# bmorris3/gadfly

Hardware: AMD Instinct MI355X
Metric: GP log-likelihood evals/sec (N=1e6, J=30) (higher is better)
Workload: dtype f64

## Files before the change

gadfly_amd/csrc/gadfly_hip.hip:

```cpp

#include <hip/hip_runtime.h>
#include <atomic>
#include <utility>
#include <type_traits>
#include <stdint.h>
#include <stdio.h>
#include <stdarg.h>
#include <math.h>

#include "../../include/gadfly_hip.h"
#include "gf_internal.h"

#define FM_INLINE __device__ __forceinline__
#include "fastmath.h"
#include "gf_wave.h"
#include "gf_sweep.h"

template <unsigned long long BITS>
__device__ __forceinline__ double fm_local_constant(const int z) {
    return __hiloint2double((int)(unsigned)(BITS >> 32) ^ z, (int)(unsigned)(BITS & 0xffffffffull) ^ z);
}
#define GF_K(x) fm_local_constant<__builtin_bit_cast(unsigned long long, (double)(x))>(fm_z)
__device__ __forceinline__ double fm_exp_local(const double x) {
    int fm_z;
// ... 822 lines not shown
constexpr int RED_NACC = 3;
constexpr int RED_BLOCK = 256;
constexpr int RED_MAXG = 512;

__host__ __device__ inline int red_groups(int64_t N) {
    int64_t g = (N + 4095) / 4096;
    if (g < 1) g = 1;
    if (g > RED_MAXG) g = RED_MAXG;
    return (int)g;
}

__device__ inline int64_t steady_rows_stored(const double *steady, int b, int64_t N, int64_t n_first) {
    const double swd = steady[(size_t)b * ST_SIZE + ST_SW];
    if (!(swd > 0.0)) return N;
    const int64_t r = (int64_t)swd - n_first;
    return r < 0 ? 0 : (r < N ? r : N);
}

__device__ __forceinline__ void red_row(const double dn, double &s1, double &mn) {
    s1 += log(dn);
    mn = fmin(mn, dn);
}
__device__ __forceinline__ void red_row_z(const double dn, const double zn, double &s2) { s2 += zn * zn / dn; }

__device__ __forceinline__ void steady_tile_sums(const double *dp, const double *zp, const int64_t N, const int64_t lim,
                                                 double *acc, const int init, const int lane) {
    if (lim == 0 && !init) return;
    const int G = red_groups(N);
    const int64_t gl = (lim + RED_BLOCK - 1) / RED_BLOCK;
    const int Gn = gl < G ? (int)gl : G;
    double a1 = 0.0, a2 = 0.0, am = INFINITY;
#pragma unroll 1
    for (int g = 0; g < Gn; ++g) {
        double t1 = 0.0, t2 = 0.0, t3 = INFINITY;
#pragma unroll 1
        for (int w = 0; w < RED_BLOCK / 64; ++w) {
            double s1 = 0.0, s2 = 0.0, mn = INFINITY;
#pragma unroll 1
            for (int64_t n = (int64_t)g * RED_BLOCK + 64 * w + lane; n < lim; n += (int64_t)G * RED_BLOCK) {
                const double dn = dp[n];
                red_row(dn, s1, mn);
                red_row_z(dn, zp[n], s2);
            }
            wave_sum2(s1, s2);
            mn = -wave_max(-mn);
            t1 += s1;
            t2 += s2;
            t3 = fmin(t3, mn);
        }
        if (lane == (g & 63)) {
            a1 += t1;
            a2 += t2;
            am = fmin(am, t3);
        }
    }
    wave_sum2(a1, a2);
    am = -wave_max(-am);
    if (lane == 0) {
        if (!init) { a1 += acc[0]; a2 += acc[1]; am = fmin(am, acc[2]); }
        acc[0] = a1; acc[1] = a2; acc[2] = am;
    }
}

template <int ROWS, bool ROWSTORE, bool SAMPLE = false, bool STEADY = false>
__global__ void __launch_bounds__(64, 2)
k_factor7(const int64_t N, const int64_t n_first, const int64_t chunk_len, const int nch,
          const int ch0, const int nsel, const int Jr, const int Jc, const int block_sub, const double gap,
          const double *__restrict__ ar_, const double *__restrict__ cr_,
          const double *__restrict__ ac_, const double *__restrict__ bc_,
          const double *__restrict__ cc_, const double *__restrict__ dc_,
          const double *__restrict__ diag_add_, const double *__restrict__ cmax_,
          const double *__restrict__ t_, const int64_t t_bs,
          const double *__restrict__ diag_, const int64_t diag_bs,
          const double *__restrict__ y_, const int64_t y_bs,
          double *__restrict__ d_, double *__restrict__ z_, double *__restrict__ r_out,
          double *__restrict__ Ut_out, double *__restrict__ Wt_out, double *__restrict__ de_out,
          double *__restrict__ S_state, double *__restrict__ F_state,
          int32_t *__restrict__ info, double *__restrict__ steady_, const int64_t arm_from,
          double *acc_, const int acc_init) {
    static_assert(!STEADY || (!ROWSTORE && !SAMPLE), "steady mode: the streamed log-likelihood only");
    const int lane = threadIdx.x;
    const int g = lane >> 5, c = lane & 31;
    const int sel = blockIdx.x;
    const int pr = sel / nsel, ch = ch0 + (sel - pr * nsel);
    const int b = pr * nch + ch;
    int64_t tile_lim = 0;
#define STEADY_EXIT(lim) do { if constexpr (STEADY) { if (acc_) { tile_lim = (lim); goto tile_sums; } } return; } while (0)
  {
    if (info[b] != 0) STEADY_EXIT(steady_rows_stored(steady_, pr, N, n_first));
    double *__restrict__ hdr = STEADY ? steady_ + (size_t)pr * ST_SIZE : nullptr;
    if constexpr (STEADY) { if (hdr[ST_SW] > 0.0) STEADY_EXIT(steady_rows_stored(steady_, pr, N, n_first)); }
    const int64_t c0 = (int64_t)ch * chunk_len;
    const int64_t rows = (N - c0 < chunk_len) ? (N - c0) : chunk_len;
    const int64_t g0 = n_first + c0;
    const size_t pb = (size_t)pr * N + c0;
    const double *__restrict__ tg = t_ + (size_t)pr * t_bs + g0;
    const double *__restrict__ yg = y_ + (size_t)pr * y_bs + g0;
    const bool has_g = diag_ != nullptr;
    const double *__restrict__ gg = has_g ? diag_ + (size_t)pr * diag_bs + g0 : yg;
    double *__restrict__ dg = d_ + pb;
    double *__restrict__ zg = SAMPLE ? z_ + (size_t)pr * y_bs + g0 : z_ + pb;
    const int own = 2 * c + g;
    double *__restrict__ rg = (ROWSTORE && r_out) ? r_out + pb * 64 + own : nullptr;
    double *__restrict__ ug = (ROWSTORE && Ut_out) ? Ut_out + pb * 64 + own : nullptr;
    double *__restrict__ wg = (ROWSTORE && Wt_out) ? Wt_out + pb * 64 + own : nullptr;
    const bool st_ok = own < ROWS || Wt_out != nullptr;
    double *__restrict__ eg = (ROWSTORE && de_out) ? de_out + pb : nullptr;
    double *__restrict__ Sg = S_state + (size_t)b * (64 * 64);
    double *__restrict__ Fg = F_state + (size_t)b * 64;
    const double diag_add = diag_add_[pr];

    RowGen G;
    G.init(own, pr, Jr, Jc, block_sub, gap, ar_, cr_, ac_, bc_, cc_, dc_, cmax_, tg, g0);
    const double cj = G.cj;

    __shared__ __attribute__((aligned(16))) double s_w[64];
    __shared__ __attribute__((aligned(16))) double s_u[64];
    __shared__ __attribute__((aligned(16))) double s_e[64];
    const double2 *pw = (const double2 *)s_w + g, *pu = (const double2 *)s_u + g;
    const double2 *pe = (const double2 *)s_e + g;
    const bool f31 = c == 31;
    const bool fl = lane == 63;
    const double not63 = fl ? 0.0 : 1.0, is31 = f31 ? 1.0 : 0.0;

    double *__restrict__ col0 = Sg + (size_t)(2 * c) * 64 + 2 * g;
    double *__restrict__ col1 = (f31 ? Fg : Sg + (size_t)(2 * c + 1) * 64) + 2 * g;
    double T[ROWS / 2][2];
    const bool zero_start = (block_sub >> 30) & 1;
    constexpr double thr = ST_THR;
    int cnt = 0, fill = 0;
    if constexpr (STEADY) {
        cnt = __builtin_amdgcn_readfirstlane((int)hdr[ST_CNT]);
        fill = __builtin_amdgcn_readfirstlane((int)hdr[ST_FILL]);
    }
#pragma unroll
    for (int m = 0; m < ROWS / 2; ++m) {
        T[m][0] = zero_start ? 0.0 : col0[4 * (m >> 1) + (m & 1)];
        T[m][1] = zero_start ? 0.0 : col1[4 * (m >> 1) + (m & 1)];
    }
    double q0 = 0.0, q1 = 0.0;
    int32_t fail = 0;

    double t_n1 = tg[1], t_n2 = tg[2];
    double y_n = yg[0], y_n1 = yg[1];
    double g_n = gg[0], g_n1 = gg[1];
    double ut, vt, de;
    bool rst;
    G.next(tg[0], g0, ut, vt, rst, de);

    double2 ub[S7_AHEAD + 1], wb[S7_AHEAD + 1];
    s_w[own] = 0.0;
    s_u[own] = ut;
    wave_lds_fence();
    sweep7_preload<ROWS>(ub, wb, pu, pw);

    int64_t n = 0;
    for (; n < rows; ++n) {
        const double a_n = (has_g ? g_n : 0.0) + diag_add, yy = y_n;
        const double ut_c = ut, vt_c = vt;
        const bool rst_c = rst;
        if constexpr (ROWSTORE) { if (eg && lane == 0) eg[n] = rst ? de : -1.0; }
        if (rst) {
            const double el = fm_exp(-cj * de);
            s_e[own] = el;
            wave_lds_fence();
            double d0, d1, el0, el1;
            both_halves(el, el0, el1);
            sweep7_preload<ROWS>(ub, wb, pe, pw);
            sweep7_run<ROWS, true>(T, ub, wb, pe, pw, q0, q1, el0, el1, d0, d1);
            sweep7_preload<ROWS>(ub, wb, pu, pw);
            q0 = 0.0;
            q1 = 0.0;
        }
        __builtin_amdgcn_s_setprio(0);
        double acc0, acc1;
        sweep7_run<ROWS, false>(T, ub, wb, pu, pw, q0, q1, 0.0, 0.0, acc0, acc1);
        __builtin_amdgcn_s_setprio(GF_CHAIN_PRIO);
        const double tmp = own_column_sum(acc0, acc1);
        const double r = (vt_c - tmp) * not63;
        double r0, r1;
        both_halves(r, r0, r1);
        G.next(t_n1, g0 + n + 1, ut, vt, rst, de);
        t_n1 = t_n2; y_n = y_n1; g_n = g_n1;
        t_n2 = tg[n + 3];
        y_n1 = yg[n + 2];
        g_n1 = gg[n + 2];
        wave_lds_fence();
        s_w[own] = r;
        s_u[own] = ut;
        wave_lds_fence();
        sweep7_preload<ROWS>(ub, wb, pu, pw);
        const double s1 = wave_sum(ut_c * tmp);
        const double s2 = read_lane(tmp, 63);
        const double dn = a_n - s1;
        const double zn = SAMPLE ? __dsqrt_rn(dn) * yy : yy - s2;
        if (!(dn > 0.0)) {
            const int64_t gf = g0 + n + 1;
            fail = (int32_t)(gf > 0x7fffffff ? 0x7fffffff : gf);
            break;
        }
        const double inv = fast_rcp(dn);
        q0 = r0 * inv;
        q1 = fma(zn, is31, r1) * inv;
        if constexpr (ROWSTORE) {
            const size_t ro = opaque_uniform((size_t)n * 64);
            if (st_ok) {
                if (rg) rg[ro] = r;
                if (ug) ug[ro] = ut_c;
                if (wg) wg[ro] = r * inv;
            }
        }
        if (lane == 0) { dg[n] = dn; zg[n] = SAMPLE ? zn + s2 : zn; }
        if constexpr (STEADY) {
            const int64_t gn = g0 + n;
            if (rst_c && gn >= arm_from && (gn & (ST_GRID - 1)) == 0) {
                double cs, sn;
                both_halves(vt_c, cs, sn);
                const double Gr = fma(r0, cs, r1 * sn) * inv, Gi = fma(r1, cs, -r0 * sn) * inv;
                const double x = fl ? dn : (g ? Gi : Gr);
                double *__restrict__ slot = hdr + ST_RING + (size_t)((gn / ST_GRID) & (ST_LAG - 1)) * 64 + lane;
                const double xo = *slot;
                *slot = x;
                const double dx = fl ? 0.0 : fabs(x - xo);
                const double mdx = wave_max(dx), mx = wave_max(fl ? 0.0 : fabs(x));
                const double dold = read_lane(xo, 63);
                const bool ok = fill >= ST_LAG && mdx <= thr * mx && fabs(dn - dold) <= thr * dn && !G.qmode;
                cnt = ok ? cnt + 1 : 0;
                fill = fill < ST_LAG ? fill + 1 : fill;
                if (lane == 0) { hdr[ST_CNT] = (double)cnt; hdr[ST_FILL] = (double)fill; }
                if (cnt >= ST_COUNT && G.dt_ref > 0.0) {
                    wave_lds_fence();
                    if (f31) {
#pragma unroll
                        for (int m = 0; m < ROWS / 2; ++m) {
                            const int i = 2 * g + 4 * (m >> 1) + (m & 1);
                            s_e[i] = fma(s_w[i], q1, T[m][1]);
                        }
                    }
                    wave_lds_fence();
                    const double F0 = (2 * c + 1 < ROWS) ? s_e[2 * c] : 0.0, F1 = (2 * c + 1 < ROWS) ? s_e[2 * c + 1] : 0.0;
                    if (g == 0) {
                        hdr[ST_GR + c] = Gr;
                        hdr[ST_GI + c] = Gi;
                        hdr[ST_SR + c] = fma(cs, F0, sn * F1);
                        hdr[ST_SI + c] = fma(cs, F1, -sn * F0);
                    }
                    if (lane == 0) {
                        hdr[ST_SW] = (double)(gn + 1);
                        hdr[ST_D] = dn;
                        hdr[ST_DT] = (tg[n] - tg[n - ST_DLAG]) * (1.0 / ST_DLAG);
                    }
                    STEADY_EXIT(n + 1);
                }
            }
        }
    }
    if (fail) {
        if (lane == 0) info[b] = fail;
        if (zero_start) {
            for (int m = 0; m < 32; ++m) {
                col0[4 * (m >> 1) + (m & 1)] = 0.0;
                col1[4 * (m >> 1) + (m & 1)] = 0.0;
            }
            if (f31)
                for (int m = 0; m < 32; ++m) Sg[63 * 64 + 2 * g + 4 * (m >> 1) + (m & 1)] = 0.0;
        }
        STEADY_EXIT(N);
    }
    wave_lds_fence();
#pragma unroll
    for (int m = 0; m < ROWS / 2; ++m) {
        const double w = s_w[2 * g + 4 * (m >> 1) + (m & 1)];
        col0[4 * (m >> 1) + (m & 1)] = fma(w, q0, T[m][0]);
        col1[4 * (m >> 1) + (m & 1)] = fma(w, q1, T[m][1]);
    }
    if (zero_start) {
        for (int m = ROWS / 2; m < 32; ++m) {
            col0[4 * (m >> 1) + (m & 1)] = 0.0;
            col1[4 * (m >> 1) + (m & 1)] = 0.0;
        }
        if (f31)
            for (int m = 0; m < 32; ++m) Sg[63 * 64 + 2 * g + 4 * (m >> 1) + (m & 1)] = 0.0;
    }
    STEADY_EXIT(N);
  }
#undef STEADY_EXIT
tile_sums:
    if constexpr (STEADY) {
        __builtin_amdgcn_s_setprio(0);
        __builtin_amdgcn_fence(__ATOMIC_RELEASE, "workgroup");
        __builtin_amdgcn_fence(__ATOMIC_ACQUIRE, "workgroup");
        steady_tile_sums(d_ + (size_t)pr * N, z_ + (size_t)pr * N, N, tile_lim, acc_ + (size_t)pr * RED_NACC, acc_init, lane);
    }
}

constexpr int STT_STAGE = 8;
constexpr int FG = 6;
__device__ __forceinline__ double wave_shr1(const double v) { return dpp_get<0x138, 0xf>(v); }
__device__ __forceinline__ void stage_end() {
    wave_lds_fence();
    __builtin_amdgcn_sched_barrier(0);
}

#define GF_MFMA64(a, b, c) __builtin_amdgcn_mfma_f64_16x16x4f64((a), (b), (c), 0, 0, 0)
typedef double d4 __attribute__((ext_vector_type(4)));

constexpr int CH_P = 64 * 64;
constexpr int CH_SLOT = 72;

template <int ROWS, bool STORE, int CHUNK = 0>
__device__ __forceinline__ void
steady_tail_rows(const int64_t N, const int64_t n_first, const int Jc, const double gap,
                 const double *__restrict__ ac_, const double *__restrict__ bc_,
                 const double *__restrict__ cc_, const double *__restrict__ dc_, const double *__restrict__ cmax_,
                 const double *__restrict__ t_, const int64_t t_bs, const double *__restrict__ y_, const int64_t y_bs,
                 double *__restrict__ d_, double *__restrict__ z_, const int32_t *__restrict__ info,
                 double *__restrict__ steady_, double *__restrict__ acc_,
                 const int64_t sw_lo, const int64_t sw_hi,
                 const int64_t chunk_rows = 0, double *__restrict__ ws_ = nullptr, const int64_t ws_ld = 0) {
    static_assert(CHUNK == 0 || !STORE, "the chunked launch stores no row");
    constexpr int JT = ROWS / 2;
    constexpr bool FOLD = !STORE;
    const int lane = threadIdx.x, pr = blockIdx.x;
    const int half = lane >> 5, tk = FOLD ? (lane & 31) : lane;
    if (info[pr] != 0) return;
    double *__restrict__ hdr = steady_ + (size_t)pr * ST_SIZE;
    const double swd = hdr[ST_SW];
    if (!(swd > 0.0)) return;
    const int64_t sw = (int64_t)swd;
    if constexpr (!STORE) { if (sw < sw_lo || sw >= sw_hi) return; }
    const int64_t nb = sw > n_first ? sw - n_first : 0;
    if (nb >= N) return;
    int64_t r_lo_ = nb, r_hi_ = N;
    int ch = 0, nch = 1;
    double *__restrict__ wsp = nullptr;
    if constexpr (CHUNK != 0) {
        ch = blockIdx.y;
        nch = (int)((N - nb + chunk_rows - 1) / chunk_rows);
        wsp = ws_ + (size_t)pr * ws_ld;
        if constexpr (CHUNK == 3) {
            if (nch < 3) return;
            r_hi_ = nb + 128 * (int64_t)Jc;
        } else {
            if (ch >= nch) return;
            if (CHUNK == 1 && ch > 0 && ch == nch - 1) return;
            if (CHUNK == 2 && ch == 0) return;
            r_lo_ = nb + ch * chunk_rows;
            r_hi_ = (N - r_lo_ > chunk_rows) ? r_lo_ + chunk_rows : N;
        }
    }
    const int64_t r_lo = r_lo_, r_hi = r_hi_;
    const double *__restrict__ tg = t_ + (size_t)pr * t_bs + n_first;
    const double *__restrict__ yg = y_ + (size_t)pr * y_bs + n_first;
    double *__restrict__ dg = STORE ? d_ + (size_t)pr * N : nullptr;
    double *__restrict__ zg = STORE ? z_ + (size_t)pr * N : nullptr;
    const double dinf = hdr[ST_D], delta = hdr[ST_DT];
    double zsq = 0.0;

    __shared__ __attribute__((aligned(16))) double s_s[64];
    __shared__ __attribute__((aligned(16))) double s_p[128];
    __shared__ __attribute__((aligned(16))) double s_h[FOLD ? 16 + 64 : 64];
    double *const hh = s_h + (FOLD ? 16 : 0);
    __shared__ __attribute__((aligned(16))) double s_z[64];
    __shared__ double s_c[STT_STAGE][2][64];
    auto taps = [&](const double *pp, double &a0, double &a1) {
#pragma unroll
        for (int m = 0; m < 64; m += 2) {
            const double2 hv = ((const double2 *)hh)[m >> 1];
            a0 = fma(hv.x, pp[-m], a0);
            a1 = fma(hv.y, pp[-m - 1], a1);
        }
    };
    auto shifted_taps = [&](double va, double vb, double &ra, double &rb) {
        double a0 = 0.0, a1 = 0.0, b0 = 0.0, b1 = 0.0;
#pragma unroll 1
        for (int m = 0; m < 64; m += 2) {
            const double2 hv = ((const double2 *)hh)[m >> 1];
            a0 = fma(hv.x, va, a0);
            b0 = fma(hv.x, vb, b0);
            va = wave_shr1(va);
            vb = wave_shr1(vb);
            a1 = fma(hv.y, va, a1);
            b1 = fma(hv.y, vb, b1);
            va = wave_shr1(va);
            vb = wave_shr1(vb);
        }
        ra = a0 + a1;
        rb = b0 + b1;
    };

    const bool term = tk < Jc;
    const size_t ck = (size_t)pr * Jc + (term ? tk : 0);
    const double ck_c = term ? cc_[ck] : 0.0, ck_d = term ? dc_[ck] : 0.0;
    const double ck_a = term ? ac_[ck] : 0.0, ck_b = term ? bc_[ck] : 0.0;
    const double wmax = wave_max(fmax(ck_c, fabs(ck_d)));
    const double gthr = gap / cmax_[pr], jthr = 2e-6 / wmax;
    double lr, li;
    {
        double sn, cs;
        fm_sincos(ck_d * delta, &sn, &cs);
        const double e = fm_exp(-ck_c * delta);
        lr = e * cs;
        li = -e * sn;
    }
    const bool gain = FOLD || lane < 32;
    const double Gr = gain ? hdr[ST_GR + (lane & 31)] : 0.0, Gi = gain ? hdr[ST_GI + (lane & 31)] : 0.0;
    double sr = (lane < 32) ? hdr[ST_SR + (lane & 31)] : 0.0, si = (lane < 32) ? hdr[ST_SI + (lane & 31)] : 0.0;
    if constexpr (CHUNK == 1) {
        if (ch > 0) { sr = 0.0; si = 0.0; }
    }
    if constexpr (CHUNK == 2) {
        const double *__restrict__ slot = wsp + CH_P;
        const double *__restrict__ prow = wsp + 64 * lane;
        double v = slot[lane];
        for (int cp = 1; cp < ch; ++cp) {
            wave_lds_fence();
            s_z[lane] = v;
            wave_lds_fence();
            double a0 = slot[cp * CH_SLOT + lane], a1 = 0.0;
#pragma unroll 4
            for (int k = 0; k < 64; k += 2) {
                const double2 vv = ((const double2 *)s_z)[k >> 1];
                a0 = fma(prow[k], vv.x, a0);
                a1 = fma(prow[k + 1], vv.y, a1);
            }
            v = a0 + a1;
        }
        wave_lds_fence();
        s_z[lane] = v;
        wave_lds_fence();
        sr = (lane < 32) ? s_z[lane] : 0.0;
        si = (lane < 32) ? s_z[lane + 32] : 0.0;
        wave_lds_fence();
    }
    const double l2r = fma(lr, lr, -li * li), l2i = 2.0 * lr * li;
    const double lgr = fma(lr, Gr, -li * Gi), lgi = fma(lr, Gi, li * Gr);
    double l32r = l2r, l32i = l2i;
    if constexpr (FOLD) {
#pragma unroll
        for (int q = 0; q < 4; ++q) {
            const double xr = fma(l32r, l32r, -l32i * l32i);
            l32i = 2.0 * l32r * l32i;
            l32r = xr;
        }
    }

    if (hdr[ST_HOK] != 0.0) {
        hh[lane] = hdr[ST_H + lane];
    } else {
        double hr = Gr, hi = Gi, hv = (lane == 0) ? 1.0 : 0.0;
        const double ha = (lane < 32) ? ck_a : 0.0, hb = (lane < 32) ? ck_b : 0.0;
        for (int m = 1; m < 64; ++m) {
            const double xr = fma(lr, hr, -li * hi), xi = fma(lr, hi, li * hr);
            const double hm = -wave_sum(fma(ha, xr, -hb * xi));
            hr = fma(Gr, hm, xr);
            hi = fma(Gi, hm, xi);
            hv = (lane == m) ? hm : hv;
        }
        hh[lane] = hv;
        if constexpr (CHUNK == 0) {
            hdr[ST_H + lane] = hv;
            if (lane == 0) hdr[ST_HOK] = 1.0;
        }
    }
    if constexpr (!FOLD) s_p[lane] = 0.0;
    else if (lane < 16) s_h[lane] = 0.0;

    double pcr[JT], pci[JT];
    const double di = delta * (double)(lane + 1);
#pragma unroll
    for (int k0 = 0; k0 < JT; k0 += STT_STAGE) {
        wave_lds_fence();
#pragma unroll 1
        for (int kk = 0; kk < STT_STAGE; ++kk) {
            const int k = k0 + kk;
            double vr = 0.0, vi = 0.0;
            if (k < Jc) {
                const size_t uk = (size_t)pr * Jc + k;
                const double a = ac_[uk], b = bc_[uk];
                double sn, cs;
                fm_sincos(dc_[uk] * di, &sn, &cs);
                const double e = fm_exp(-cc_[uk] * di);
                vr = -e * fma(a, cs, b * sn);
                vi = e * fma(b, cs, -a * sn);
                if constexpr (FOLD) shifted_taps(vr, vi, vr, vi);
            }
            s_c[kk][0][lane] = vr;
            s_c[kk][1][lane] = vi;
        }
        wave_lds_fence();
#pragma unroll
        for (int kk = 0; kk < STT_STAGE; ++kk) {
            if (k0 + kk < JT) { pcr[k0 + kk] = s_c[kk][0][lane]; pci[k0 + kk] = s_c[kk][1][lane]; }
        }
    }

    const int64_t last = N - 1;
    auto row_of = [&](const int64_t cb) { const int64_t i = cb + lane; return i < last ? i : last; };
    bool viol = false;
    double t_nx = tg[row_of(r_lo)], tp_nx = tg[row_of(r_lo) - 1];
    auto add_term = [&](const int k, const double2 sv, double &x0, double &x1) {
        if (k & 1) x1 = fma(pci[k], sv.y, fma(pcr[k], sv.x, x1));
        else x0 = fma(pci[k], sv.y, fma(pcr[k], sv.x, x0));
    };
    auto two_rows = [&](const double2 zz) {
        const double wr = fma(lgr, zz.x, Gr * zz.y), wi = fma(lgi, zz.x, Gi * zz.y);
        const double nr = fma(l2r, sr, fma(-l2i, si, wr));
        si = fma(l2r, si, fma(l2i, sr, wi));
        sr = nr;
    };
    auto one_row = [&](const double zj) {
        const double nr = fma(lr, sr, fma(-li, si, Gr * zj));
        si = fma(lr, si, fma(li, sr, Gi * zj));
        sr = nr;
    };
    if constexpr (!FOLD) {
    double y_nx = yg[row_of(nb)];
    for (int64_t cb = nb; cb < N; cb += 64) {
        const double yv = y_nx, tv = t_nx, tp = tp_nx;
        {
            const int64_t i = row_of(cb + 64);
            y_nx = yg[i]; t_nx = tg[i]; tp_nx = tg[i - 1];
        }
        const int lim = (int)(N - cb < 64 ? N - cb : 64);
        const double dt = tv - tp;
        viol |= (lane < lim) && ((dt > gthr) || !(fabs(dt - delta) < jthr));
        wave_lds_fence();
        if (lane < 32) { s_s[2 * lane] = sr; s_s[2 * lane + 1] = si; }
        wave_lds_fence();
        double p0 = yv, p1 = 0.0;
#pragma unroll
        for (int k = 0; k < JT; ++k) add_term(k, ((const double2 *)s_s)[k], p0, p1);
        s_p[64 + lane] = p0 + p1;
        wave_lds_fence();
        double z0 = 0.0, z1 = 0.0;
        taps(s_p + 64 + lane, z0, z1);
        const double zv = z0 + z1;
        s_z[lane] = zv;
        wave_lds_fence();
        if (lane < lim) { dg[cb + lane] = dinf; zg[cb + lane] = zv; }
        int j = 0;
#pragma unroll 4
        for (; j + 1 < lim; j += 2) two_rows(((const double2 *)s_z)[j >> 1]);
        if (j < lim) one_row(s_z[j]);
    }
    } else {
    constexpr int SU = 64 + 1;
    __shared__ __attribute__((aligned(16))) double s_u[16 * SU];
    const int mc = lane & 15, mk = lane >> 4;
    auto group_phase = [&](const int64_t g0) {
        double ha[4][4];
#pragma unroll
        for (int d = 0; d < 4; ++d)
#pragma unroll
            for (int q = 0; q < 4; ++q) ha[d][q] = hh[16 * d + mc - 4 * q - mk];
        d4 U[4];
#pragma unroll
        for (int I = 0; I < 4; ++I) U[I] = d4{0.0, 0.0, 0.0, 0.0};
        const int64_t r0 = g0 + 64 * mc + mk;
#pragma unroll
        for (int Jt = 0; Jt < 4; ++Jt) {
            double yb[4];
#pragma unroll
            for (int q = 0; q < 4; ++q) {
                const int64_t i = r0 + 16 * Jt + 4 * q;
                yb[q] = yg[i < last ? i : last];
            }
#pragma unroll
            for (int q = 0; q < 4; ++q)
#pragma unroll
                for (int I = Jt; I < 4; ++I) U[I] = GF_MFMA64(ha[I - Jt][q], yb[q], U[I]);
        }
        wave_lds_fence();
#pragma unroll
        for (int I = 0; I < 4; ++I)
#pragma unroll
            for (int r = 0; r < 4; ++r) s_u[mc * SU + 16 * I + mk + 4 * r] = U[I][r];
        wave_lds_fence();
    };
    const double *zb = s_z + 32 * half;
    auto join = [&](const double jr, const double ji) {
        double slr, sur, sli, sui;
        both_halves(sr, slr, sur);
        both_halves(si, sli, sui);
        sr = half ? 0.0 : fma(jr, slr, fma(-ji, sli, sur));
        si = half ? 0.0 : fma(jr, sli, fma(ji, slr, sui));
    };
    int64_t cb = r_lo;
    if constexpr (CHUNK == 3) {
        for (int i = lane; i < 16 * SU; i += 64) s_u[i] = 0.0;
        for (int i = lane; i < 64 * (32 - Jc); i += 64) {
            const int r = i / (32 - Jc), k = Jc + i % (32 - Jc);
            wsp[64 * r + k] = 0.0;
            wsp[64 * r + 32 + k] = 0.0;
        }
        wave_lds_fence();
    }
    while (cb < r_hi) {
    if constexpr (CHUNK != 3) group_phase(cb);
    const double *ub = s_u + lane;
    const int64_t ge = (r_hi - cb > 16 * 64) ? cb + 16 * 64 : r_hi;
    for (; cb + 64 <= ge; cb += 64, ub += SU) {
        if constexpr (CHUNK == 3) {
            const int j = (int)((cb - r_lo) >> 6);
            sr = (j < Jc && lane == j) ? 1.0 : 0.0;
            si = (j >= Jc && lane == j - Jc) ? 1.0 : 0.0;
        } else {
        const double tv = t_nx, tp = tp_nx;
        {
            const int64_t i = row_of(cb + 64);
            t_nx = tg[i]; tp_nx = tg[i - 1];
        }
        const double dt = tv - tp;
        viol |= (dt > gthr) || !(fabs(dt - delta) < jthr);
        }
        wave_lds_fence();
        if (lane < 32) { s_s[2 * lane] = sr; s_s[2 * lane + 1] = si; }
        wave_lds_fence();
        constexpr int NG = (JT + FG - 1) / FG;
        double z0 = *ub, z1 = 0.0;
        double2 sv[2][FG], zz[16];
        auto s_ld = [&](const int g) {
#pragma unroll
            for (int i = 0; i < FG; ++i)
                if (g * FG + i < JT) sv[g & 1][i] = ((const double2 *)s_s)[g * FG + i];
        };
        s_ld(0);
#pragma unroll
        for (int g = 0; g < NG; ++g) {
            if (g + 1 < NG) s_ld(g + 1);
            stage_end();
#pragma unroll
            for (int i = 0; i < FG; ++i) {
                const int k = g * FG + i;
                if (k < JT) add_term(k, sv[g & 1][i], z0, z1);
            }
        }
        const double zv = z0 + z1;
        s_z[lane] = zv;
        wave_lds_fence();
        zsq = fma(zv, zv, zsq);
#pragma unroll
        for (int i = 0; i < 8; ++i) zz[i] = ((const double2 *)zb)[i];
#pragma unroll
        for (int j2 = 0; j2 < 16; ++j2) {
            if (j2 >= 4 && j2 < 12 && (j2 & 3) == 0) {
#pragma unroll
                for (int i = j2 + 4; i < j2 + 8; ++i) zz[i] = ((const double2 *)zb)[i];
            }
            stage_end();
            two_rows(zz[j2]);
        }
        join(l32r, l32i);
        if constexpr (CHUNK == 3) {
            if (lane < 32) {
                const int j = (int)((cb - r_lo) >> 6), col = j < Jc ? j : 32 + j - Jc;
                wsp[64 * lane + col] = sr;
                wsp[64 * (32 + lane) + col] = si;
            }
        }
    }
    if (cb < ge) {
        const int lim = (int)(r_hi - cb);
        const double dt = t_nx - tp_nx;
        viol |= (lane < lim) && ((dt > gthr) || !(fabs(dt - delta) < jthr));
        wave_lds_fence();
        if (lane < 32) { s_s[2 * lane] = sr; s_s[2 * lane + 1] = si; }
        wave_lds_fence();
        double z0 = *ub, z1 = 0.0;
#pragma unroll
        for (int k = 0; k < JT; ++k) {
            add_term(k, ((const double2 *)s_s)[k], z0, z1);
            if (k % FG == FG - 1) stage_end();
        }
        const double zv = z0 + z1;
        s_z[lane] = zv;
        wave_lds_fence();
        zsq = (lane < lim) ? fma(zv, zv, zsq) : zsq;
        const int mine = half ? (lim > 32 ? lim - 32 : 0) : (lim < 32 ? lim : 32);
        int j = 0;
#pragma unroll 1
        for (; j + 1 < mine; j += 2) two_rows(((const double2 *)zb)[j >> 1]);
        if (j < mine) one_row(zb[j]);
        double jr = 1.0, ji = 0.0;
        for (int q = 32; q < lim; ++q) {
            const double xr = fma(jr, lr, -ji * li);
            ji = fma(jr, li, ji * lr);
            jr = xr;
        }
        join(jr, ji);
        cb = r_hi;
    }
    }
    }
    if constexpr (CHUNK != 0) {
        if constexpr (CHUNK == 3) return;
        if (__ballot(viol) != 0ull && lane == 0) hdr[ST_VIOL] = 1.0;
        double *__restrict__ slot = wsp + CH_P + ch * CH_SLOT;
        if (ch == nch - 1) {
            if (lane < 32) { hdr[ST_SR + lane] = sr; hdr[ST_SI + lane] = si; }
        } else if (CHUNK == 1 && lane < 32) {
            slot[lane] = sr;
            slot[32 + lane] = si;
        }
        if (CHUNK == 2 || ch == 0) {
            const double q = wave_sum(zsq);
            if (lane == 0) slot[64] = q;
        }
        return;
    }
    if (lane < 32) { hdr[ST_SR + lane] = sr; hdr[ST_SI + lane] = si; }
    if (__ballot(viol) != 0ull && lane == 0) hdr[ST_VIOL] = 1.0;
    if constexpr (!STORE) {
        const double q = wave_sum(zsq);
        if (lane == 0) {
            double *__restrict__ a = acc_ + (size_t)pr * RED_NACC;
            a[0] += (double)(N - nb) * log(dinf);
            a[1] += q / dinf;
            a[2] = fmin(a[2], dinf);
        }
    }
}

template <int ROWS>
__global__ void __launch_bounds__(64, 2)
k_steady_tail(const int64_t N, const int64_t n_first, const int Jc, const double gap,
              const double *__restrict__ ac_, const double *__restrict__ bc_,
              const double *__restrict__ cc_, const double *__restrict__ dc_, const double *__restrict__ cmax_,
              const double *__restrict__ t_, const int64_t t_bs, const double *__restrict__ y_, const int64_t y_bs,
              double *__restrict__ d_, double *__restrict__ z_, const int32_t *__restrict__ info,
              double *__restrict__ steady_) {
    steady_tail_rows<ROWS, true>(N, n_first, Jc, gap, ac_, bc_, cc_, dc_, cmax_, t_, t_bs, y_, y_bs, d_, z_, info,
                                 steady_, nullptr, 0, 0);
}

template <int ROWS>
__global__ void __launch_bounds__(64, 2)
k_steady_finish(const int64_t N, const int Jc, const double gap,
                const double *__restrict__ ac_, const double *__restrict__ bc_,
                const double *__restrict__ cc_, const double *__restrict__ dc_, const double *__restrict__ cmax_,
                const double *__restrict__ t_, const int64_t t_bs, const double *__restrict__ y_, const int64_t y_bs,
                const int32_t *__restrict__ info, double *__restrict__ steady_, double *__restrict__ acc_,
                const int64_t sw_lo, const int64_t sw_hi) {
    steady_tail_rows<ROWS, false>(N, 0, Jc, gap, ac_, bc_, cc_, dc_, cmax_, t_, t_bs, y_, y_bs, nullptr, nullptr, info,
                                  steady_, acc_, sw_lo, sw_hi);
}

template <int ROWS, int PASS>
__global__ void __launch_bounds__(64, 2)
k_steady_chunk(const int64_t N, const int Jc, const double gap,
               const double *__restrict__ ac_, const double *__restrict__ bc_,
               const double *__restrict__ cc_, const double *__restrict__ dc_, const double *__restrict__ cmax_,
               const double *__restrict__ t_, const int64_t t_bs, const double *__restrict__ y_, const int64_t y_bs,
               const int32_t *__restrict__ info, double *__restrict__ steady_,
               const int64_t sw_lo, const int64_t sw_hi, const int64_t chunk_rows, double *__restrict__ ws_,
               const int64_t ws_ld) {
    steady_tail_rows<ROWS, false, PASS>(N, 0, Jc, gap, ac_, bc_, cc_, dc_, cmax_, t_, t_bs, y_, y_bs, nullptr, nullptr,
                                        info, steady_, nullptr, sw_lo, sw_hi, chunk_rows, ws_, ws_ld);
}

__device__ __forceinline__ int64_t steady_chunk_problem(const int pr, const int64_t N, const int32_t *__restrict__ info,
                                                        const double *__restrict__ steady_, const int64_t sw_lo,
                                                        const int64_t sw_hi, const int64_t chunk_rows, const int least) {
    if (info[pr] != 0) return 0;
    const double swd = steady_[(size_t)pr * ST_SIZE + ST_SW];
    if (!(swd > 0.0)) return 0;
    const int64_t sw = (int64_t)swd;
    if (sw < sw_lo || sw >= sw_hi || sw >= N) return 0;
    return (N - sw + chunk_rows - 1) / chunk_rows >= least ? sw : 0;
}

__global__ void __launch_bounds__(256)
k_steady_chunk_power(const int64_t N, const int32_t *__restrict__ info, const double *__restrict__ steady_,
                     const int64_t sw_lo, const int64_t sw_hi, const int64_t chunk_rows, const int squarings,
                     double *__restrict__ ws_, const int64_t ws_ld) {
    const int pr = blockIdx.x;
    if (steady_chunk_problem(pr, N, info, steady_, sw_lo, sw_hi, chunk_rows, 3) == 0) return;
    __shared__ double s_m[64][64 + 1];
    double *__restrict__ P = ws_ + (size_t)pr * ws_ld;
    const int i = threadIdx.x >> 2, c0 = 16 * (threadIdx.x & 3);
    double a[16];
#pragma unroll
    for (int j = 0; j < 16; ++j) a[j] = P[64 * i + c0 + j];
    for (int q = 0; q < squarings; ++q) {
        __syncthreads();
#pragma unroll
        for (int j = 0; j < 16; ++j) s_m[i][c0 + j] = a[j];
        __syncthreads();
#pragma unroll
        for (int j = 0; j < 16; ++j) a[j] = 0.0;
#pragma unroll 4
        for (int k = 0; k < 64; ++k) {
            const double m = s_m[i][k];
#pragma unroll
            for (int j = 0; j < 16; ++j) a[j] = fma(m, s_m[k][c0 + j], a[j]);
        }
    }
#pragma unroll
    for (int j = 0; j < 16; ++j) P[64 * i + c0 + j] = a[j];
}

__global__ void __launch_bounds__(64)
k_steady_chunk_sum(const int B, const int64_t N, const int32_t *__restrict__ info, const double *__restrict__ steady_,
                   const int64_t sw_lo, const int64_t sw_hi, const int64_t chunk_rows,
                   const double *__restrict__ ws_, const int64_t ws_ld, double *__restrict__ acc_) {
    const int pr = blockIdx.x * 64 + threadIdx.x;
    if (pr >= B) return;
    const int64_t sw = steady_chunk_problem(pr, N, info, steady_, sw_lo, sw_hi, chunk_rows, 1);
    if (sw == 0) return;
    const int nch = (int)((N - sw + chunk_rows - 1) / chunk_rows);
    const double *__restrict__ slot = ws_ + (size_t)pr * ws_ld + CH_P;
    double q = 0.0;
    for (int c = 0; c < nch; ++c) q += slot[c * CH_SLOT + 64];
    const double dinf = steady_[(size_t)pr * ST_SIZE + ST_D];
    double *__restrict__ a = acc_ + (size_t)pr * RED_NACC;
    a[0] += (double)(N - sw) * log(dinf);
    a[1] += q / dinf;
    a[2] = fmin(a[2], dinf);
}

constexpr int R1_RR = 0, R1_RI = 64, R1_YR = 128, R1_YI = 192, R1_XR = 256, R1_XI = 320;
constexpr int R1_D = 384, R1_SG = 385;

__device__ __forceinline__ void half_wave_sums(double v, double &lo, double &up) {
    v += dpp_get<0xB1, 0xf>(v);
    v += dpp_get<0x4E, 0xf>(v);
    v += dpp_get<0x141, 0xf>(v);
    v += dpp_get<0x140, 0xf>(v);
    v += dpp_get<0x142, 0xf>(v);
    lo = read_lane(v, 31);
    up = read_lane(v, 63);
}

__device__ __forceinline__ double lane_select(const unsigned long long lanes, const double v, const double keep) {
    int lo = __double2loint(keep), hi = __double2hiint(keep);
    asm("v_cndmask_b32 %0, %0, %1, %2" : "+v"(lo) : "v"(__double2loint(v)), "s"(lanes));
    asm("v_cndmask_b32 %0, %0, %1, %2" : "+v"(hi) : "v"(__double2hiint(v)), "s"(lanes));
    return __hiloint2double(hi, lo);
}

constexpr int R1_UNROLL = 8;

__global__ void __launch_bounds__(64, 2)
k_steady_rank1(const int64_t N, const int64_t n_first, const int Jc, const double gap,
               const double *__restrict__ ac_, const double *__restrict__ bc_,
               const double *__restrict__ cc_, const double *__restrict__ dc_,
               const double *__restrict__ diag_add_, const double *__restrict__ cmax_,
               const double *__restrict__ t_, const int64_t t_bs,
               const double *__restrict__ diag_, const int64_t diag_bs,
               const double *__restrict__ y_, const int64_t y_bs,
               double *__restrict__ d_, double *__restrict__ z_, double *__restrict__ S_state,
               int32_t *__restrict__ info, double *__restrict__ steady_, const int64_t arm_from,
               const double *__restrict__ dt_, double *acc_, const int acc_init) {
    const int lane = threadIdx.x, pr = blockIdx.x;
    const int h = lane >> 5, c = lane & 31;
    int64_t tile_lim = 0;
#define R1_EXIT(lim) do { if (acc_) { tile_lim = (lim); goto tile_sums; } return; } while (0)
  {
    if (info[pr] != 0) R1_EXIT(steady_rows_stored(steady_, pr, N, n_first));
    double *__restrict__ hdr = steady_ + (size_t)pr * ST_SIZE;
    if (hdr[ST_SW] > 0.0) R1_EXIT(steady_rows_stored(steady_, pr, N, n_first));
    const double *__restrict__ tg = t_ + (size_t)pr * t_bs + n_first;
    const double *__restrict__ yg = y_ + (size_t)pr * y_bs + n_first;
    double *__restrict__ dg = d_ + (size_t)pr * N;
    double *__restrict__ zg = z_ + (size_t)pr * N;
    double *__restrict__ Sg = S_state + (size_t)pr * (64 * 64);
    const bool term = c < Jc, fl = lane == 63;
    const size_t ck = (size_t)pr * Jc + (term ? c : 0);
    const double ck_c = term ? cc_[ck] : 0.0, ck_d = term ? dc_[ck] : 0.0;
    const double ck_a = term ? ac_[ck] : 0.0, ck_b = term ? bc_[ck] : 0.0;
    const double wmax = wave_max(fmax(ck_c, fabs(ck_d)));
    const double gthr = gap / cmax_[pr], jthr = 2e-6 / wmax;
    const double delta = dt_[pr];
    double lr, li;
    {
        double sn, cs;
        fm_sincos(ck_d * delta, &sn, &cs);
        const double e = fm_exp(-ck_c * delta);
        lr = e * cs;
        li = -e * sn;
    }
    double rr, ri, Yr, Yi, Xr, Xi, d, sg;
    if (n_first == 0) {
        d = (diag_ ? diag_[(size_t)pr * diag_bs] : 0.0) + diag_add_[pr];
        sg = fast_rcp(d);
        rr = term ? 1.0 : 0.0;
        ri = 0.0;
        Yr = term ? lr : 0.0;
        Yi = term ? li : 0.0;
        Xr = h ? Yr : 0.0;
        Xi = h ? Yi : 0.0;
    } else {
        rr = Sg[R1_RR + lane]; ri = Sg[R1_RI + lane];
        Yr = Sg[R1_YR + lane]; Yi = Sg[R1_YI + lane];
        Xr = Sg[R1_XR + lane]; Xi = Sg[R1_XI + lane];
        d = Sg[R1_D]; sg = Sg[R1_SG];
    }
    constexpr double thr = ST_THR;
    int cnt = __builtin_amdgcn_readfirstlane((int)hdr[ST_CNT]);
    int fill = __builtin_amdgcn_readfirstlane((int)hdr[ST_FILL]);
    int32_t fail = 0;
    double inv = fast_rcp(d);
    double kr = rr * inv, ki = ri * inv;
    const int64_t last = N - 1;
    auto row_of = [&](const int64_t cb) { const int64_t i = cb + lane; return i < last ? i : last; };
    double t_nx, tp_nx, y_nx;
    {
        const int64_t i = row_of(0);
        t_nx = tg[i];
        tp_nx = (n_first + i > 0) ? tg[i - 1] : t_nx - delta;
        y_nx = yg[i];
    }
    double sd = 0.0, sz = 0.0, sr, si, beta, yv_blk = 0.0;
    auto row_front = [&](const int j) __attribute__((always_inline)) {
        const double yy = read_lane(yv_blk, j);
        double sf;
        half_wave_sums(fma(ck_a, Xr, -(ck_b * Xi)), sf, beta);
        const double zn = yy - sf;
        const unsigned long long row_lane = 1ull << j;
        sd = lane_select(row_lane, d, sd);
        sz = lane_select(row_lane, zn, sz);
        const double m = h ? -beta : zn;
        sr = fma(kr, m, Xr), si = fma(ki, m, Xi);
    };
    auto row_back = [&]() __attribute__((always_inline)) {
        Xr = fma(lr, sr, -(li * si));
        Xi = fma(lr, si, li * sr);
        const double sb = sg * beta;
        rr = fma(-sb, Yr, rr);
        ri = fma(-sb, Yi, ri);
        const double dn = fma(-sb, beta, d);
        const double wr = fma(-beta, kr, Yr), wi = fma(-beta, ki, Yi);
        Yr = fma(lr, wr, -(li * wi));
        Yi = fma(lr, wi, li * wr);
        inv = fast_rcp(dn);
        sg = sg * d * inv;
        d = dn;
        kr = rr * inv;
        ki = ri * inv;
    };
    auto plain_rows = [&](int j, const int j1) __attribute__((always_inline)) {
        for (; j + R1_UNROLL <= j1; j += R1_UNROLL) {
#pragma unroll
            for (int u = 0; u < R1_UNROLL; ++u) {
                row_front(j + u);
                row_back();
            }
        }
#pragma unroll 1
        for (; j < j1; ++j) {
            row_front(j);
            row_back();
        }
    };
    auto first_failed = [&](const int rows) __attribute__((always_inline)) {
        const unsigned long long staged = rows < 64 ? (1ull << rows) - 1 : ~0ull;
        const unsigned long long bad = __ballot(!(sd > 0.0)) & staged;
        return bad ? (int)__ffsll((long long)bad) - 1 : -1;
    };
    auto flush = [&](const int64_t nb, const int rows) __attribute__((always_inline)) {
        if (lane < rows) { dg[nb + lane] = sd; zg[nb + lane] = sz; }
    };
    const int g0lo = (int)(n_first & (ST_GRID - 1));
    const int ja = (ST_GRID - g0lo) & (ST_GRID - 1);
    __builtin_amdgcn_s_setprio(GF_CHAIN_PRIO);
    for (int64_t nb = 0; nb < N; nb += 64) {
        const int lim = (int)(N - nb < 64 ? N - nb : 64);
        yv_blk = y_nx;
        asm volatile("" : "+v"(yv_blk));
        {
            const double dt = t_nx - tp_nx;
            const bool bad = (dt > gthr) || !(fabs(dt - delta) < jthr);
            if (__any(bad) && lane == 0) hdr[ST_VIOL] = 1.0;
            const int64_t i = row_of(nb + 64);
            t_nx = tg[i];
            tp_nx = (n_first + i > 0) ? tg[i - 1] : t_nx - delta;
            y_nx = yg[i];
        }
        int jf;
        if (ja < lim) {
            plain_rows(0, ja);
            row_front(ja);
            jf = first_failed(ja + 1);
            if (jf < 0) {
                const int64_t n = nb + ja, gn = n_first + n;
                if (gn >= arm_from) {
// ... 4119 lines not shown
```

Baseline: 51210.

## Fold steady-state recurrence four rows per step with double-double powers of lambda

For the folded steady-tail path with ROWS<64, the complex scan recurrence now advances four rows per step instead of two. It does this using precomputed lambda^2..lambda^4 and G-scaled powers, which are computed in double-double so the longer jumps lose no accuracy. This shortens the serial dependency chain through the per-lane state. The add_term loop is also paired so each step feeds two independent accumulators. The cost is extra setup arithmetic and more registers, and the reassociation may change rounding slightly.

Result: faster. 54080 (median of 6 runs) (+5.6%).

```diff
diff --git a/gadfly_amd/csrc/gadfly_hip.hip b/gadfly_amd/csrc/gadfly_hip.hip
--- a/gadfly_amd/csrc/gadfly_hip.hip
+++ b/gadfly_amd/csrc/gadfly_hip.hip
@@ -1148,6 +1148,30 @@
     __builtin_amdgcn_sched_barrier(0);
 }
 
+struct cdd { double rh, rl, ih, il; };
+__device__ __forceinline__ void dd_sum(const double a, const double b, double &s, double &e) {
+#pragma clang fp contract(off)
+    s = a + b;
+    const double bb = s - a;
+    e = (a - (s - bb)) + (b - bb);
+}
+__device__ __forceinline__ void dd_pair(const double a1, const double b1, const double a2, const double b2, const double sg,
+                                        const double tail, double &hi, double &lo) {
+#pragma clang fp contract(off)
+    const double p1 = a1 * b1, e1 = fma(a1, b1, -p1);
+    const double p2 = sg * (a2 * b2), e2 = sg * fma(a2, b2, -(a2 * b2));
+    double s, es;
+    dd_sum(p1, p2, s, es);
+    const double l = es + ((e1 + e2) + tail);
+    dd_sum(s, l, hi, lo);
+}
+__device__ __forceinline__ cdd cdd_mul(const cdd a, const cdd b) {
+    cdd c;
+    dd_pair(a.rh, b.rh, a.ih, b.ih, -1.0, fma(a.rh, b.rl, a.rl * b.rh) - fma(a.ih, b.il, a.il * b.ih), c.rh, c.rl);
+    dd_pair(a.rh, b.ih, a.ih, b.rh, 1.0, fma(a.rh, b.il, a.rl * b.ih) + fma(a.ih, b.rl, a.il * b.rh), c.ih, c.il);
+    return c;
+}
+
 #define GF_MFMA64(a, b, c) __builtin_amdgcn_mfma_f64_16x16x4f64((a), (b), (c), 0, 0, 0)
 typedef double d4 __attribute__((ext_vector_type(4)));
 
@@ -1167,6 +1191,7 @@
     static_assert(CHUNK == 0 || !STORE, "the chunked launch stores no row");
     constexpr int JT = ROWS / 2;
     constexpr bool FOLD = !STORE;
+    constexpr bool FOUR = FOLD && ROWS < 64;
     const int lane = threadIdx.x, pr = blockIdx.x;
     const int half = lane >> 5, tk = FOLD ? (lane & 31) : lane;
     if (info[pr] != 0) return;
@@ -1432,6 +1457,33 @@
         sr = half ? 0.0 : fma(jr, slr, fma(-ji, sli, sur));
         si = half ? 0.0 : fma(jr, sli, fma(ji, slr, sui));
     };
+    double l4r = 0.0, l4i = 0.0, g1r = 0.0, g1i = 0.0, g2r = 0.0, g2i = 0.0, g3r = 0.0, g3i = 0.0;
+    if constexpr (FOUR) {
+        const cdd l1{lr, 0.0, li, 0.0}, gd{Gr, 0.0, Gi, 0.0};
+        const cdd l2 = cdd_mul(l1, l1), l3 = cdd_mul(l2, l1), l4 = cdd_mul(l2, l2);
+        cdd lp = l4;
+#pragma unroll
+        for (int q = 0; q < 3; ++q) lp = cdd_mul(lp, lp);
+        const cdd g1 = cdd_mul(l1, gd), g2 = cdd_mul(l2, gd), g3 = cdd_mul(l3, gd);
+        l4r = l4.rh; l4i = l4.ih;
+        l32r = lp.rh; l32i = lp.ih;
+        g1r = g1.rh; g1i = g1.ih; g2r = g2.rh; g2i = g2.ih; g3r = g3.rh; g3i = g3.ih;
+    }
+    auto add_pair = [&](const int k, const double2 sa, const double2 sb, double &x0, double &x1) {
+        x0 = fma(pcr[k], sa.x, x0);
+        x1 = fma(pcr[k + 1], sb.x, x1);
+        x0 = fma(pci[k], sa.y, x0);
+        x1 = fma(pci[k + 1], sb.y, x1);
+    };
+    auto four_w = [&](const double2 za, const double2 zc, double &wr, double &wi) {
+        wr = fma(g3r, za.x, fma(g2r, za.y, fma(g1r, zc.x, Gr * zc.y)));
+        wi = fma(g3i, za.x, fma(g2i, za.y, fma(g1i, zc.x, Gi * zc.y)));
+    };
+    auto four_s = [&](const double wr, const double wi) {
+        const double nr = fma(l4r, sr, fma(-l4i, si, wr));
+        si = fma(l4r, si, fma(l4i, sr, wi));
+        sr = nr;
+    };
     int64_t cb = r_lo;
     if constexpr (CHUNK == 3) {
         for (int i = lane; i < 16 * SU; i += 64) s_u[i] = 0.0;
@@ -1477,9 +1529,9 @@
             if (g + 1 < NG) s_ld(g + 1);
             stage_end();
 #pragma unroll
-            for (int i = 0; i < FG; ++i) {
+            for (int i = 0; i < FG; i += 2) {
                 const int k = g * FG + i;
-                if (k < JT) add_term(k, sv[g & 1][i], z0, z1);
+                if (k < JT) add_pair(k, sv[g & 1][i], sv[g & 1][i + 1], z0, z1);
             }
         }
         const double zv = z0 + z1;
@@ -1488,6 +1540,24 @@
         zsq = fma(zv, zv, zsq);
 #pragma unroll
         for (int i = 0; i < 8; ++i) zz[i] = ((const double2 *)zb)[i];
+        if constexpr (FOUR) {
+            double wr, wi;
+            stage_end();
+            four_w(zz[0], zz[1], wr, wi);
+#pragma unroll
+            for (int t = 0; t < 8; ++t) {
+                if (t == 1 || t == 3) {
+#pragma unroll
+                    for (int i = 6 + 2 * t; i < 10 + 2 * t; ++i) zz[i] = ((const double2 *)zb)[i];
+                }
+                stage_end();
+                double nwr = 0.0, nwi = 0.0;
+                if (t < 7) four_w(zz[2 * t + 2], zz[2 * t + 3], nwr, nwi);
+                four_s(wr, wi);
+                wr = nwr;
+                wi = nwi;
+            }
+        } else {
 #pragma unroll
         for (int j2 = 0; j2 < 16; ++j2) {
             if (j2 >= 4 && j2 < 12 && (j2 & 3) == 0) {
@@ -1496,6 +1566,7 @@
             }
             stage_end();
             two_rows(zz[j2]);
+        }
         }
         join(l32r, l32i);
         if constexpr (CHUNK == 3) {
@@ -1525,9 +1596,20 @@
         zsq = (lane < lim) ? fma(zv, zv, zsq) : zsq;
         const int mine = half ? (lim > 32 ? lim - 32 : 0) : (lim < 32 ? lim : 32);
         int j = 0;
+        if constexpr (FOUR) {
+#pragma unroll 1
+            for (; j + 3 < mine; j += 4) {
+                double wr, wi;
+                four_w(((const double2 *)zb)[j >> 1], ((const double2 *)zb)[(j >> 1) + 1], wr, wi);
+                four_s(wr, wi);
+            }
+#pragma unroll 1
+            for (; j < mine; ++j) one_row(zb[j]);
+        } else {
 #pragma unroll 1
         for (; j + 1 < mine; j += 2) two_rows(((const double2 *)zb)[j >> 1]);
         if (j < mine) one_row(zb[j]);
+        }
         double jr = 1.0, ji = 0.0;
         for (int q = 32; q < lim; ++q) {
             const double xr = fma(jr, lr, -ji * li);
```
